# epam/Zstandard

Hardware: NVIDIA B200
Metric: decompress_GBps_uncompressed (higher is better)
Workload: dtype u8

## Files before the change

### zstandard_b200/csrc/decode_kernels.cu

```cuda
#include "zb_decode.cuh"
#include "decode_kernels.cuh"
#include "xxh_device.cuh"
#ifdef ZB_EXEC_DEBUG
#include <stdio.h>
#endif

namespace zb {

__device__ __forceinline__ u64 frame_dst_off(const DecodeArgs& a, u32 f, const FrameInfo& fi) { return a.dst_off[f] + fi.out_base; }
__device__ __forceinline__ u32 frame_cap(const DecodeArgs& a, u32 f, const FrameInfo& fi) { return a.dst_cap[f] - fi.out_base; }
__device__ __forceinline__ u8* lit_region(const DecodeArgs& a, u32 f, const FrameInfo& fi) { return a.lit_arena + (frame_dst_off(a, f, fi) & ~15ull) + 64ull * (a.item_base + f); }
__device__ __forceinline__ u64 lit_capacity(u32 cap) { return (u64)cap + 40; }
__device__ __forceinline__ SeqRec* seq_region(const DecodeArgs& a, u32 f, const FrameInfo& fi) { return a.seq_arena + 2 * (frame_dst_off(a, f, fi) / 3) + 32ull * (a.item_base + f); }

__device__ __forceinline__ u64 unit_slice_base(const DecodeArgs& a) { return a.dst_off[0] / PAR_UNIT_BYTES + (u64)PAR_UNIT_SLACK * a.item_base; }

__device__ __forceinline__ int parse_one(const DecodeArgs& a, u32 i) {
  FrameInfo fi; u32 r = 0; u32 start = 0, outBase = 0;
  if (a.pass) {
    const FrameInfo prev = a.info[i];
    if ((prev.flags & FI_DONE) || prev.next_off == 0 || is_err(a.result[i])) { a.info[i].flags = FI_DONE; return -1; }
    start = prev.next_off; outBase = prev.out_base + prev.decoded;
  }
  const u8* src = a.src_base + a.src_off[i];
// ... 120 lines not shown
          if (ok) ok = huf_build_tables(sm, slot, sub, gmask, body, bodySize, fullMem, T, &hdr);
          if (ok) { body += hdr; bodySize -= hdr; haveTable = true; }
        }
        if (ok) {
          bool good = true;
          if (lh.single) {
            if (sub == 0) good = dry ? huf_check_stream(body, bodySize, lh.litSize, T)
                                     : huf_decode_stream(body, bodySize, lit + litRun, lh.litSize, T, &sm.ring[lane][0]);
          } else {
            HufStream st;
            good = huf_split4(body, bodySize, lh.litSize, sub, st);
            if (good) good = dry ? huf_check_stream(st.src, st.len, st.count, T)
                                 : huf_decode_stream(st.src, st.len, lit + litRun + st.outOfs, st.count, T, &sm.ring[lane][0]);
          }
          unsigned okmask = __ballot_sync(gmask, good);
          if ((okmask & gmask) != gmask) ok = false;
          __syncwarp(gmask);
        }
        if (!ok || dry) { errBlock = blk; errCode = ok ? HUF_DRY : ZE_corruption_detected; break; }
        litRun += lh.litSize;
      }
    }
    pos += bh.csize; blk++;
    if (bh.last) break;
  }
  if (sub == 0 && errBlock != 0xFFFFFFFFu) { a.info[f].huf_err_block = errBlock; a.info[f].huf_err_code = errCode; }
}

template <int R>
__global__ void __launch_bounds__(32) k_huf(DecodeArgs a) {
  extern __shared__ __align__(16) unsigned char smem_raw[];
  HufSmem<R>& sm = *reinterpret_cast<HufSmem<R>*>(smem_raw);
  const u32 lane = threadIdx.x, slot = lane >> 2;
  const u32 nSmall = a.cnt[2];
  if (R == (int)HUF_ROOT_SMALL ? nSmall == 0 : nSmall == a.n) return;
  u16* const fullMem = a.huf_full + (size_t)(blockIdx.x * 8 + slot) * HUF_FULL_STRIDE;
  for (u32 g = blockIdx.x; g * 8 < a.n; g += gridDim.x) {
    const u32 f = g * 8 + slot;
    if (f < a.n) huf_frame(a, sm, f, lane, fullMem);
  }
}

template <int CL, int CO, int CM> struct SeqSmemT {
  u16 ll[1 << CL][32];
  u16 ml[1 << CM][32];
  u16 of[1 << CO][32];
  u16 defLL[64], defOF[32], defML[64];
  u32 llInfo[36], mlInfo[53];
  s16 norm[53][32];
  u16 next[53][32];
  __align__(16) u32 ring[32][ZB_RING_WORDS + 4];
};
typedef SeqSmemT<9, 8, 9> SeqSmem;

template <class SM>
__device__ __forceinline__ void seq_smem_init(SM& sm, u32 lane) {
  if (lane < 3) {
    s16* norm = &sm.norm[0][lane]; u16* next = &sm.next[0][lane];
    Strided<s16> nv{norm, 32}; Strided<u16> sn{next, 32};
    if (lane == 0) { for (int i = 0; i < 36; i++) nv[i] = kLLnorm[i]; build_seq_table(sm.defLL, 1, nv, 35, 6, sn); }
    if (lane == 1) { for (int i = 0; i < 29; i++) nv[i] = kOFnorm[i]; build_seq_table(sm.defOF, 1, nv, 28, 5, sn); }
    if (lane == 2) { for (int i = 0; i < 53; i++) nv[i] = kMLnorm[i]; build_seq_table(sm.defML, 1, nv, 52, 6, sn); }
  }
  for (u32 i = lane; i < 36; i += 32) sm.llInfo[i] = ll_info(i);
  for (u32 i = lane; i < 53; i += 32) sm.mlInfo[i] = ml_info(i);
  __syncwarp();
}

template <int CLS, int CL, int CO, int CM>
__global__ void __launch_bounds__(32) k_seq_t(DecodeArgs a) {
  extern __shared__ __align__(16) unsigned char smem_raw[];
  typedef SeqSmemT<CL, CO, CM> SM;
  SM& sm = *reinterpret_cast<SM*>(smem_raw);
  const u32 lane = threadIdx.x;
  const u32 k = CLS == 0 ? 2 : CLS - 1;
  const u32 count = a.cnt[3 + k];
  if (blockIdx.x * 32 >= count) return;
  seq_smem_init(sm, lane);
  const u32 e = blockIdx.x * 32 + lane;
  if (e >= count) return;
  const u32 f = a.par_list[(size_t)(1 + k) * a.list_stride + a.item_base + e];
  const FrameInfo fi = a.info[f];
  SeqTableSet T;
  T.cap[KIND_LL] = CL; T.cap[KIND_OF] = CO; T.cap[KIND_ML] = CM;
  T.space[KIND_LL] = &sm.ll[0][lane]; T.space[KIND_ML] = &sm.ml[0][lane]; T.space[KIND_OF] = &sm.of[0][lane]; T.stride = 32;
  T.defs[KIND_LL] = sm.defLL; T.defs[KIND_OF] = sm.defOF; T.defs[KIND_ML] = sm.defML;
  SeqEmitter em;
  em.init(seq_region(a, f, fi), seq_capacity(frame_cap(a, f, fi)), sm.llInfo, sm.mlInfo);
  if (a.dict) em.set_reps(a.dict->rep);
  seq_decode_frame(a.src_base + a.src_off[f], a.src_size[f], fi.body_off, fi.window, T, em, sm.llInfo, sm.mlInfo,
                   Strided<s16>{&sm.norm[0][lane], 32}, Strided<u16>{&sm.next[0][lane], 32}, &sm.ring[lane][0], a.dict);
  if (CLS != 0 && em.deferred) {
    a.info[f].flags = fi.flags & ~(u32)(FI_SEQ_A | FI_SEQ_B);
    a.par_list[(size_t)3 * a.list_stride + a.item_base + atomicAdd(a.cnt + 5, 1u)] = f;
    return;
  }
  if (em.res.err_block != 0xFFFFFFFFu) {
    a.info[f].seq_err_block = em.res.err_block; a.info[f].seq_err_code = em.res.err_code; a.info[f].seq_err_index = em.res.err_index;
  }
}

__device__ __forceinline__ void warp_copy(u8* dst, const u8* src, u32 n, u32 lane) {
  if (n < 128) { for (u32 i = lane; i < n; i += 32) dst[i] = src[i]; return; }
  u32 head = (u32)(-(intptr_t)dst) & 15;
  if (lane < head) dst[lane] = src[lane];
  dst += head; src += head; n -= head;
  u32 body = n & ~15u;
  if ((((uintptr_t)src) & 15) == 0) {
    const uint4* s = (const uint4*)src; uint4* d = (uint4*)dst;
    for (u32 i = lane; i < body / 16; i += 32) d[i] = s[i];
  } else {
    const u32 sh = ((u32)(uintptr_t)src & 3) * 8;
    const u32* s = (const u32*)((uintptr_t)src & ~(uintptr_t)3); uint4* d = (uint4*)dst;
    for (u32 i = lane; i < body / 16; i += 32) {
      const u32* p = s + 4 * i;
      u32 w0 = p[0], w1 = p[1], w2 = p[2], w3 = p[3], w4 = sh ? p[4] : 0;
      d[i] = make_uint4(__funnelshift_r(w0, w1, sh), __funnelshift_r(w1, w2, sh), __funnelshift_r(w2, w3, sh), __funnelshift_r(w3, w4, sh));
    }
  }
  for (u32 i = body + lane; i < n; i += 32) dst[i] = src[i];
}
__device__ __forceinline__ void warp_fill(u8* dst, u8 v, u32 n, u32 lane) {
  if (n < 128) { for (u32 i = lane; i < n; i += 32) dst[i] = v; return; }
  u32 head = (u32)(-(intptr_t)dst) & 15;
  if (lane < head) dst[lane] = v;
  dst += head; n -= head;
  u32 body = n & ~15u, w = v * 0x01010101u;
  uint4* d = (uint4*)dst; uint4 vv = make_uint4(w, w, w, w);
  for (u32 i = lane; i < body / 16; i += 32) d[i] = vv;
  for (u32 i = body + lane; i < n; i += 32) dst[i] = v;
}

// ... 309 lines not shown
__global__ void __launch_bounds__(32) k_huf_blk(DecodeArgs a) {
  extern __shared__ __align__(16) unsigned char smem_raw[];
  HufSmem<HUF_TABLE_LOG>& sm = *reinterpret_cast<HufSmem<HUF_TABLE_LOG>*>(smem_raw);
  const u32 lane = threadIdx.x, sub = lane & 3, slot = lane >> 2;
  const unsigned gmask = 0xFu << (slot * 4);
  const u32 nunits = a.cnt[0];
  BlockUnit* const sliceUnits = a.units + unit_slice_base(a);
  u16* const fullMem = a.huf_full + (size_t)(blockIdx.x * 8 + slot) * HUF_FULL_STRIDE;
  for (u32 w0 = blockIdx.x * 8; w0 < nunits; w0 += gridDim.x * 8) {
    const u32 w = w0 + slot;
    if (w >= nunits) continue;
    const BlockUnit u = sliceUnits[w];
    const u32 f = u.frame;
    const FrameInfo fi = a.info[f];
    const u8* src = a.src_base + a.src_off[f];
    const u8* bp = src + u.body;
    LitHdr lh; bool needs;
    read_lit_hdr(bp, u.csize, lh, &needs);
    if (lh.type < 2) continue;
    u8* lit = lit_region(a, f, fi) + u.lit_off;
    bool ok = true;
    HufTabs T{sm.root[slot], HUF_TABLE_LOG, nullptr, nullptr, 0};
    const u8* body = bp + lh.lhSize; u32 bodySize = lh.litCSize;
    __syncwarp(gmask);
    if (lh.type == 3 && u.huf_def == DEF_DICT) huf_dict_tables(sm, slot, sub, gmask, a.dict, T);
    else {
      const u8* tb = body; u32 tbSize = bodySize;
      if (lh.type == 3) {
        const BlockUnit d = sliceUnits[fi.unit_base + u.huf_def];
        LitHdr lhD; bool n2;
        read_lit_hdr(src + d.body, d.csize, lhD, &n2);
        tb = src + d.body + lhD.lhSize; tbSize = lhD.litCSize;
      } else if (!lh.single && (lh.litSize == 0 || bodySize == 0)) ok = false;
      u32 hdr = 0;
      if (ok) ok = huf_build_tables(sm, slot, sub, gmask, tb, tbSize, fullMem, T, &hdr);
      if (ok && lh.type == 2) { body += hdr; bodySize -= hdr; }
    }
    if (ok) {
      bool good = true;
      if (lh.single) {
        if (sub == 0) good = huf_decode_stream(body, bodySize, lit, lh.litSize, T, &sm.ring[lane][0]);
      } else {
        HufStream st;
        good = huf_split4(body, bodySize, lh.litSize, sub, st);
        if (good) good = huf_decode_stream(st.src, st.len, lit + st.outOfs, st.count, T, &sm.ring[lane][0]);
      }
      const unsigned okmask = __ballot_sync(gmask, good);
      if ((okmask & gmask) != gmask) ok = false;
    }
    if (sub == 0 && !ok) sliceUnits[w].huf_err = ZE_corruption_detected;
  }
}

__global__ void __launch_bounds__(32) k_seq_blk(DecodeArgs a) {
  extern __shared__ __align__(16) unsigned char smem_raw[];
  SeqSmem& sm = *reinterpret_cast<SeqSmem*>(smem_raw);
  const u32 lane = threadIdx.x;
  const u32 nunits = a.cnt[0];
  if (blockIdx.x * 32 >= nunits) return;
  if (lane < 3) {
    s16* norm = &sm.norm[0][lane]; u16* next = &sm.next[0][lane];
    Strided<s16> nv{norm, 32}; Strided<u16> sn{next, 32};
    if (lane == 0) { for (int i = 0; i < 36; i++) nv[i] = kLLnorm[i]; build_seq_table(sm.defLL, 1, nv, 35, 6, sn); }
    if (lane == 1) { for (int i = 0; i < 29; i++) nv[i] = kOFnorm[i]; build_seq_table(sm.defOF, 1, nv, 28, 5, sn); }
    if (lane == 2) { for (int i = 0; i < 53; i++) nv[i] = kMLnorm[i]; build_seq_table(sm.defML, 1, nv, 52, 6, sn); }
  }
  for (u32 i = lane; i < 36; i += 32) sm.llInfo[i] = ll_info(i);
  for (u32 i = lane; i < 53; i += 32) sm.mlInfo[i] = ml_info(i);
  __syncwarp();
  BlockUnit* const sliceUnits = a.units + unit_slice_base(a);
  for (u32 w = blockIdx.x * 32 + lane; w < nunits; w += gridDim.x * 32) {
    const BlockUnit u = sliceUnits[w];
    const u32 f = u.frame;
    const FrameInfo fi = a.info[f];
    SeqTableSet T;
    T.space[KIND_LL] = &sm.ll[0][lane]; T.space[KIND_ML] = &sm.ml[0][lane]; T.space[KIND_OF] = &sm.of[0][lane]; T.stride = 32;
    T.defs[KIND_LL] = sm.defLL; T.defs[KIND_OF] = sm.defOF; T.defs[KIND_ML] = sm.defML;
    UnitEmitter em;
    em.init(seq_region(a, f, fi) + u.rec_off, sm.llInfo, sm.mlInfo);
    seq_decode_unit(a.src_base + a.src_off[f], u, sliceUnits + fi.unit_base, fi.window, T, em, sm.llInfo, sm.mlInfo,
                    Strided<s16>{&sm.norm[0][lane], 32}, Strided<u16>{&sm.next[0][lane], 32}, &sm.ring[lane][0], a.dict);
    if (em.dead) { sliceUnits[w].seq_err_code = em.err_code; sliceUnits[w].seq_err_index = em.err_index; }
    else if (em.n) {
      sliceUnits[w].rep[0] = em.h.v0; sliceUnits[w].rep[1] = em.h.v1; sliceUnits[w].rep[2] = em.h.v2;
      sliceUnits[w].rep_sym = em.h.t0 | (em.h.t1 << 3) | (em.h.t2 << 6);
    }
  }
}

#ifndef EXECB_SLEEP
#define EXECB_SLEEP 100
#endif
__host__ __device__ inline u32 execb_warps(u32 npar) { return npar <= 148 * 7 ? 4 : (npar <= 148 * 16 ? 2 : 1); }
template <int W> struct ExecBigShared {
  volatile u32 wm;
  volatile u32 done;
  volatile u32 errG;
  volatile u32 flag[4 * W];
  volatile u32 endPos[4 * W];
  u32 errAt[W], errCode[W];
  volatile u32 left;
  u32 hashed; u64 hv[4];
};
template <int W>
__device__ __forceinline__ void chain_publish(ExecBigShared<W>& sh, u32 G, u32 endPos, u32 lane) {
  __threadfence_block();
  __syncwarp();
  if (lane == 0) {
    if (W == 1) { sh.wm = endPos; sh.done = G + 1; }
    else {
      sh.endPos[G % (4 * W)] = endPos;
      __threadfence_block();
      sh.flag[G % (4 * W)] = G + 1;
      __threadfence_block();
      u32 d = sh.done;
      while (sh.flag[d % (4 * W)] == d + 1) {
        const u32 e = sh.endPos[d % (4 * W)];
        if (atomicCAS((u32*)&sh.done, d, d + 1) == d) atomicMax((u32*)&sh.wm, e);
        __threadfence_block();
        d = sh.done;
      }
    }
  }
  __syncwarp();
// ... 271 lines not shown
      }
      a.result[f] = res;
      a.info[f].trailer_off = trailer; a.info[f].decoded = (u32)op; a.info[f].next_off = nextOff;
      a.info[f].flags = fi.flags | (needXxh ? FI_NEED_XXH : 0);
      if (nextOff && a.more) atomicAdd(a.more, 1u);
    }
  }
}

__global__ void __launch_bounds__(128) k_xxh(DecodeArgs a) {
  const u32 t = blockIdx.x * blockDim.x + threadIdx.x;
  const u32 f = t >> 2, sub = t & 3, lane = threadIdx.x & 31;
  const unsigned gmask = 0xFu << (lane & ~3u);
  if (f >= a.n) return;
  FrameInfo fi = a.info[f];
  if (!(fi.flags & FI_NEED_XXH) || (fi.flags & FI_PAR)) return;
  const u8* dst = a.dst_base + frame_dst_off(a, f, fi);
  u64 h = xxh64_group<false>(dst, fi.decoded, sub, gmask, lane & ~3u);
  if (sub == 0) {
    const u8* src = a.src_base + a.src_off[f];
    if ((u32)h != ld32(src + fi.trailer_off)) a.result[f] = zerr(ZE_checksum_wrong);
  }
}
__global__ void __launch_bounds__(32) k_xxh_big(DecodeArgs a) {
  const u32 lane = threadIdx.x, sub = lane & 3, slot = lane >> 2;
  const unsigned gmask = 0xFu << (lane & ~3u);
  const u32 npar = a.cnt[1];
  for (u32 p = blockIdx.x * 8 + slot; p < npar; p += gridDim.x * 8) {
    const u32 f = a.par_list[a.item_base + p];
    const FrameInfo fi = a.info[f];
    if (!(fi.flags & FI_NEED_XXH)) continue;
    const u8* dst = a.dst_base + frame_dst_off(a, f, fi);
    const u64 h = xxh64_group<true>(dst, fi.decoded, sub, gmask, lane & ~3u);
    if (sub == 0) {
      const u8* src = a.src_base + a.src_off[f];
      if ((u32)h != ld32(src + fi.trailer_off)) a.result[f] = zerr(ZE_checksum_wrong);
    }
  }
}


size_t decode_lit_arena_bytes(u64 max_dst_bytes, u64 max_items) { return (size_t)(max_dst_bytes + 64 * (max_items + 2) + 256); }
size_t decode_seq_arena_bytes(u64 max_dst_bytes, u64 max_items) { return (size_t)((2 * (max_dst_bytes / 3) + 32 * (max_items + 2) + 64) * sizeof(SeqRec)); }

__global__ void __launch_bounds__(32) k_dict(const u8* dict, u32 size, DictState* ds) {
  __shared__ HufBuildWk wk; __shared__ HufFseScratch fs; __shared__ u8 slot[260]; __shared__ s16 norm[64]; __shared__ u16 next[64];
  if (threadIdx.x == 0) dict_load(dict, size, *ds, wk, fs, slot, norm, next);
}
cudaError_t decode_load_dictionary(const u8* d_dict_bytes, u32 size, DictState* d_state, cudaStream_t st) {
  k_dict<<<1, 32, 0, st>>>(d_dict_bytes, size, d_state);
  return cudaGetLastError();
}

static int g_par_grid_huf = 148 * 5, g_grid_huf_small = 148 * 11, g_par_grid_seq = 148 * 2, g_par_grid_exec = 148 * 32;
int decode_huf_ctas() { return g_grid_huf_small > g_par_grid_huf ? g_grid_huf_small : g_par_grid_huf; }
size_t decode_unit_arena_count(u64 max_dst_bytes, u64 max_items) { return (size_t)(max_dst_bytes / PAR_UNIT_BYTES + PAR_UNIT_SLACK * (max_items + 2) + 64); }

cudaError_t decode_configure() {
  cudaError_t e = cudaFuncSetAttribute(k_huf<HUF_TABLE_LOG>, cudaFuncAttributeMaxDynamicSharedMemorySize, (int)sizeof(HufSmem<HUF_TABLE_LOG>));
  if (e != cudaSuccess) return e;
  e = cudaFuncSetAttribute(k_huf<HUF_ROOT_SMALL>, cudaFuncAttributeMaxDynamicSharedMemorySize, (int)sizeof(HufSmem<HUF_ROOT_SMALL>));
  if (e != cudaSuccess) return e;
  e = cudaFuncSetAttribute(k_huf_blk, cudaFuncAttributeMaxDynamicSharedMemorySize, (int)sizeof(HufSmem<HUF_TABLE_LOG>));
  if (e != cudaSuccess) return e;
  e = cudaFuncSetAttribute(k_seq_blk, cudaFuncAttributeMaxDynamicSharedMemorySize, (int)sizeof(SeqSmem));
  if (e != cudaSuccess) return e;
  int dev = 0, sms = 0;
  if (cudaGetDevice(&dev) == cudaSuccess && cudaDeviceGetAttribute(&sms, cudaDevAttrMultiProcessorCount, dev) == cudaSuccess && sms > 0) {
    int per = 0;
    if (cudaOccupancyMaxActiveBlocksPerMultiprocessor(&per, k_huf_blk, 32, sizeof(HufSmem<HUF_TABLE_LOG>)) == cudaSuccess && per > 0) g_par_grid_huf = sms * per;
    if (cudaOccupancyMaxActiveBlocksPerMultiprocessor(&per, k_huf<HUF_ROOT_SMALL>, 32, sizeof(HufSmem<HUF_ROOT_SMALL>)) == cudaSuccess && per > 0) g_grid_huf_small = sms * per;
    if (cudaOccupancyMaxActiveBlocksPerMultiprocessor(&per, k_seq_blk, 32, sizeof(SeqSmem)) == cudaSuccess && per > 0) g_par_grid_seq = sms * per;
    g_par_grid_exec = sms * 32;
  }
  e = cudaFuncSetAttribute(k_seq_t<2, 8, 8, 8>, cudaFuncAttributeMaxDynamicSharedMemorySize, (int)sizeof(SeqSmemT<8, 8, 8>));
  if (e != cudaSuccess) return e;
  return cudaFuncSetAttribute(k_seq_t<0, 9, 8, 9>, cudaFuncAttributeMaxDynamicSharedMemorySize, (int)sizeof(SeqSmem));
}

const char* const kDecodeKernelNames[DECODE_KERNELS] = {"k_parse", "k_huf", "k_seq", "k_exec", "k_xxh"};

cudaError_t decode_launch_entropy(const DecodeArgs& a, cudaStream_t st, int* launches, cudaEvent_t* marks) {
  if (a.n == 0) return cudaSuccess;
  { cudaError_t e = cudaMemsetAsync(a.cnt, 0, 32, st); if (e != cudaSuccess) return e; }
  if (marks) cudaEventRecord(marks[0], st);
  k_parse<<<(a.n + 127) / 128, 128, 0, st>>>(a);
  if (marks) cudaEventRecord(marks[1], st);
  { const u32 need = (a.n + 7) / 8;
    k_huf<HUF_ROOT_SMALL><<<need < (u32)g_grid_huf_small ? need : (u32)g_grid_huf_small, 32, sizeof(HufSmem<HUF_ROOT_SMALL>), st>>>(a);
    k_huf<HUF_TABLE_LOG><<<need < (u32)g_par_grid_huf ? need : (u32)g_par_grid_huf, 32, sizeof(HufSmem<HUF_TABLE_LOG>), st>>>(a); }
  if (a.units) k_huf_blk<<<g_par_grid_huf, 32, sizeof(HufSmem<HUF_TABLE_LOG>), st>>>(a);
  if (marks) cudaEventRecord(marks[2], st);
  k_seq_t<1, 6, 6, 7><<<(a.n + 31) / 32, 32, sizeof(SeqSmemT<6, 6, 7>), st>>>(a);
  k_seq_t<2, 8, 8, 8><<<(a.n + 31) / 32, 32, sizeof(SeqSmemT<8, 8, 8>), st>>>(a);
  k_seq_t<0, 9, 8, 9><<<(a.n + 31) / 32, 32, sizeof(SeqSmem), st>>>(a);
  if (a.units) k_seq_blk<<<g_par_grid_seq, 32, sizeof(SeqSmem), st>>>(a);
  if (marks) cudaEventRecord(marks[3], st);
  if (launches) *launches += a.units ? 8 : 6;
  return cudaGetLastError();
}
cudaError_t decode_launch_exec(const DecodeArgs& a, cudaStream_t st, int* launches, cudaEvent_t* marks) {
  if (a.n == 0) return cudaSuccess;
  if (a.dict) k_exec<true><<<(a.n + (EXEC_THREADS / 32) - 1) / (EXEC_THREADS / 32), EXEC_THREADS, 0, st>>>(a);
  else k_exec<false><<<(a.n + (EXEC_THREADS / 32) - 1) / (EXEC_THREADS / 32), EXEC_THREADS, 0, st>>>(a);
  if (a.units) {
    if (a.dict) {
      k_exec_big<true, 4><<<g_par_grid_exec / 32 * 7, 160, 0, st>>>(a); k_exec_big<true, 2><<<g_par_grid_exec / 2, 64, 0, st>>>(a); k_exec_big<true, 1><<<g_par_grid_exec, 32, 0, st>>>(a);
    } else {
      k_exec_big<false, 4><<<g_par_grid_exec / 32 * 7, 160, 0, st>>>(a); k_exec_big<false, 2><<<g_par_grid_exec / 2, 64, 0, st>>>(a); k_exec_big<false, 1><<<g_par_grid_exec, 32, 0, st>>>(a);
    }
  }
  if (marks) cudaEventRecord(marks[4], st);
  k_xxh<<<(a.n * 4 + 127) / 128, 128, 0, st>>>(a);
  if (a.units) k_xxh_big<<<148 * 8, 32, 0, st>>>(a);
  if (marks) cudaEventRecord(marks[5], st);
  if (launches) *launches += a.units ? 6 : 2;
  return cudaGetLastError();
}
cudaError_t decode_launch(const DecodeArgs& a, cudaStream_t st, int* launches, cudaEvent_t* marks) {
  cudaError_t e = decode_launch_entropy(a, st, launches, marks);
  if (e != cudaSuccess) return e;
  return decode_launch_exec(a, st, launches, marks);
}

}
```

### zstandard_b200/csrc/zb_blocks.cuh

```cuda
#pragma once
#include "zb_decode.cuh"

namespace zb {

enum : u32 { DEF_SELF = 0xFFFFFFFEu, DEF_DICT = 0xFFFFFFFDu, DEF_NONE = 0xFFFFFFFFu };

#define PAR_UNIT_BYTES 16384u
#define PAR_UNIT_SLACK 2u

struct BlockUnit {
  u32 frame;
  u32 body;
  u32 csize;
  u32 lit_off;
  u32 rec_off;
  u32 huf_def;
  u32 tab_def[3];
  u32 huf_err;
  u32 seq_err_code, seq_err_index;
  u32 rep[3];
  u32 rep_sym;
};
static_assert(sizeof(BlockUnit) == 64, "BlockUnit layout");

// ... 89 lines not shown
        if (lh.type == 3) u.huf_def = lastHuf; else lastHuf = n;
        litRun += lh.litSize;
      }
      if (nbSeq) {
        const int kinds[3] = {KIND_LL, KIND_OF, KIND_ML};
        const u32 modeOf[3] = {(modes >> 4) & 3, (modes >> 2) & 3, modes & 3};
        for (int k = 0; k < 3; k++) {
          if (modeOf[k] == 3) { if (lastTab[kinds[k]] == DEF_NONE) return 0; u.tab_def[kinds[k]] = lastTab[kinds[k]]; }
          else lastTab[kinds[k]] = n;
        }
        recRun += 1 + (u64)nbSeq;
        if (recRun > recCap) return 0;
      }
      if (units) units[n] = u;
      n++;
    }
    pos += bh.csize;
    if (bh.last) break;
  }
  return n >= 2 ? n : 0;
}

template <class NormT>
ZB_HD bool unit_locate_table(const u8* bp, u32 bsz, int kind, NormT norm, const u8** desc, u32* descSize, u32* mode) {
  LitHdr lh; bool needs;
  if (read_lit_hdr(bp, bsz, lh, &needs)) return false;
  const u8* sp = bp + lh.consumed; const u32 ssz = bsz - lh.consumed;
  u32 nbSeq, modes, hdr;
  if (read_seq_count(sp, ssz, &nbSeq, &modes, &hdr) || !nbSeq) return false;
  const int kinds[3] = {KIND_LL, KIND_OF, KIND_ML};
  const u32 modeOf[3] = {(modes >> 4) & 3, (modes >> 2) & 3, modes & 3};
  for (int k = 0; k < 3; k++) {
    if (kinds[k] == kind) { *desc = sp + hdr; *descSize = ssz - hdr; *mode = modeOf[k]; return true; }
    if (modeOf[k] == 1) { if (ssz - hdr == 0) return false; hdr += 1; }
    else if (modeOf[k] == 2) {
      u32 max = kinds[k] == KIND_LL ? MaxLL : (kinds[k] == KIND_ML ? MaxML : MaxOff), tl, h;
      if (read_ncount(norm, &max, &tl, sp + hdr, ssz - hdr, &h)) return false;
      hdr += h;
    }
  }
  return false;
}

template <class NormT, class NextT>
ZB_HD void seq_decode_unit(const u8* src, const BlockUnit& u, const BlockUnit* frameUnits, u64 window, SeqTableSet& T, UnitEmitter& em,
                           const u32* llInfo, const u32* mlInfo, NormT norm, NextT symbolNext, u32* ringMem, const DictState* dict) {
  const u8* bp = src + u.body; const u32 bsz = u.csize;
  LitHdr lh; bool needs;
  read_lit_hdr(bp, bsz, lh, &needs);
  const u8* sp = bp + lh.consumed; const u32 ssz = bsz - lh.consumed;
  u32 nbSeq, modes, hdr;
  read_seq_count(sp, ssz, &nbSeq, &modes, &hdr);
  if (!nbSeq) return;
  for (int k = 0; k < 3; k++) { T.cur[k] = T.space[k]; T.curStride[k] = T.stride; T.log[k] = 0; }
  const int kinds[3] = {KIND_LL, KIND_OF, KIND_ML};
  const u32 modeOf[3] = {(modes >> 4) & 3, (modes >> 2) & 3, modes & 3};
  u32 e = 0;
  for (int k = 0; k < 3 && !e; k++) {
    const int kind = kinds[k]; u32 used = 0, lg = 0; bool isDef = false;
    if (modeOf[k] == 3) continue;
    e = read_seq_table(modeOf[k], kind, sp + hdr, ssz - hdr, T.space[kind], T.stride, &lg, &isDef, true, &used, norm, symbolNext);
    if (!e) { hdr += used; T.log[kind] = lg; if (isDef) { T.cur[kind] = T.defs[kind]; T.curStride[kind] = 1; } }
  }
  for (int k = 0; k < 3 && !e; k++) {
    const int kind = kinds[k];
    if (modeOf[k] != 3) continue;
    const u32 def = u.tab_def[kind];
    if (def == DEF_DICT) {
      const u32 cells = 1u << dict->log[kind];
      for (u32 c = 0; c < cells; c++) T.space[kind][c * T.stride] = dict->cells[kind][c];
      T.log[kind] = dict->log[kind];
    } else {
      const BlockUnit& d = frameUnits[def];
      const u8* desc; u32 descSize, mode, used = 0, lg = 0; bool isDef = false;
      if (!unit_locate_table(src + d.body, d.csize, kind, norm, &desc, &descSize, &mode)) { e = ZE_corruption_detected; break; }
      e = read_seq_table(mode, kind, desc, descSize, T.space[kind], T.stride, &lg, &isDef, true, &used, norm, symbolNext);
      if (!e) { T.log[kind] = lg; if (isDef) { T.cur[kind] = T.defs[kind]; T.curStride[kind] = 1; } }
    }
  }
  if (e) { em.fail(0, ZE_corruption_detected); return; }
  seq_decode_bitstream(sp + hdr, ssz - hdr, nbSeq, window, T, em, llInfo, mlInfo, ringMem, 0);
}

}
```

### zstandard_b200/csrc/zb_decode.cuh

```cuda
#pragma once
#include "zb_format.cuh"

namespace zb {

struct alignas(16) SeqRec { u32 x, y, z, w; };
ZB_HD void rec_store(SeqRec* p, u32 x, u32 y, u32 z, u32 w) {
#if defined(__CUDA_ARCH__)
  *reinterpret_cast<uint4*>(p) = make_uint4(x, y, z, w);
#else
  p->x = x; p->y = y; p->z = z; p->w = w;
#endif
}
ZB_HD u32 rec_ll(const SeqRec& r) { return r.w & 0x1FFFF; }
ZB_HD u32 rec_ml(const SeqRec& r) { return (r.w >> 17) | (((r.y >> 18) & 7) << 15); }
ZB_HD u32 rec_lpos(const SeqRec& r) { return r.y & 0x3FFFF; }
ZB_HD u32 sat_add32(u32 a, u32 b) { const u32 s = a + b; return s < a ? 0xFFFFFFFFu : s; }
ZB_HD u32 sat_lpos(u32 lpos, u32 ll) { const u32 s = lpos + ll; return s > 0x3FFFFu ? 0x3FFFFu : s; }

ZB_HD u64 seq_capacity(u64 cap) { return 2 * (cap / 3) + 24; }

struct SeqTableSet {
  u32 cap[3] = {9, 9, 9};
  u16* space[3];
  u32 stride;
  const u16* defs[3];
  const u16* cur[3]; u32 curStride[3]; u32 log[3];
};

struct SeqFrameOut {
  u32 err_block, err_code, err_index;
};

ZB_HD u32 top_bits(u64 w, u32 n) { return (u32)((w >> 1) >> (63 - n)); }

ZB_HD u32 rep_resolve(u32& rep0, u32& rep1, u32& rep2, u32 ofBits, u32 ofv, u32 llSym) {
  const bool isRep = ofBits <= 1;
  const u32 raw = (1u << (ofBits & 31)) - 3 + ofv;
  const u32 idx = ofBits + ofv + (llSym == 0);
  u32 pick = rep0;
  pick = idx == 1 ? rep1 : pick;
  pick = idx == 2 ? rep2 : pick;
  pick = idx == 3 ? rep0 - 1 : pick;
  pick = pick == 0 ? 1 : pick;
  const u32 offset = isRep ? pick : raw;
  const bool keep1 = isRep && idx == 0;
  const bool keep2 = isRep && idx <= 1;
  const u32 n2 = keep2 ? rep2 : rep1, n1 = keep1 ? rep1 : rep0;
  rep2 = n2; rep1 = n1; rep0 = offset;
  return offset;
}

struct RefBits {
  const u8* s; u32 n;
  i32 k;
  u32 bc, C;
};
ZB_HD void refbits_load(RefBits& b) {
  if (b.n >= 4) { b.C = ld32(b.s + b.k); return; }
  b.C = b.s[0]; if (b.n >= 2) b.C |= (u32)b.s[1] << 8; if (b.n >= 3) b.C |= (u32)b.s[2] << 16;
}
ZB_HD void refbits_at(RefBits& b, const u8* s, u32 n, i32 P) {
  b.s = s; b.n = n;
  const i32 bcn = (8 - (P & 7)) & 7, above = P - 32 + bcn;
  if (n >= 4 && above >= 0) { b.k = above >> 3; b.bc = (u32)bcn; } else { b.k = 0; b.bc = (u32)(32 - P); }
  refbits_load(b);
}
ZB_HD u32 refbits_read_fast(RefBits& b, u32 nb) { u32 v = (b.C << (b.bc & 31)) >> ((32 - nb) & 31); b.bc += nb; return v; }
ZB_HD void refbits_reload(RefBits& b) {
  if (b.bc > 32 || b.k == 0) return;
  u32 nb = b.bc >> 3;
  if (b.k >= 4 || (i32)nb <= b.k) { b.k -= (i32)nb; b.bc -= nb * 8; } else { b.bc -= (u32)b.k * 8; b.k = 0; }
  refbits_load(b);
}
ZB_HD void seq_values_ref32(const u8* s, u32 n, i32 P, bool longOffsets, bool longVariant, u32 ofBits, u32 mlBits, u32 llBits, u32& ofv, u32& mlv, u32& llv) {
  RefBits b; refbits_at(b, s, n, P);
  ofv = 0;
  if (ofBits) {
    if (longOffsets && (longVariant || ofBits >= 25)) {
      const u32 room = longVariant ? 24 : 32 - b.bc, extra = ofBits - (ofBits < room ? ofBits : room);
      ofv = refbits_read_fast(b, ofBits - extra) << (extra & 31);
// ... 6 lines not shown
  llv = llBits ? refbits_read_fast(b, llBits) : 0;
}

struct SeqEmitter {
  SeqRec* out; u32 cap; const u32* llInfo; const u32* mlInfo;
  u32 n;
  u32 hdrSlot, dpos, lpos;
  u32 rep0, rep1, rep2;
  bool dead;
  bool deferred;
  SeqFrameOut res;
  ZB_HD void init(SeqRec* o, u64 cap64, const u32* lli, const u32* mli) {
    out = o; cap = (u32)cap64; llInfo = lli; mlInfo = mli;
    n = 0; hdrSlot = 0; dpos = 0; lpos = 0; rep0 = 1; rep1 = 4; rep2 = 8; dead = false; deferred = false;
    res.err_block = 0xFFFFFFFFu; res.err_code = 0; res.err_index = 0;
  }
  ZB_HD void set_reps(const u32* r) { rep0 = r[0]; rep1 = r[1]; rep2 = r[2]; }
  ZB_HD void block_begin() { if (dead) return; hdrSlot = n++; dpos = 0; lpos = 0; }
  ZB_HD void emit(u32 ofBits, u32 ofv, u32 llSym, u32 ll, u32 ml) {
    const u32 offset = rep_resolve(rep0, rep1, rep2, ofBits, ofv, llSym);
    if (n < cap) rec_store(out + n, dpos, lpos | ((ml >> 15) << 18), offset, ll | (ml << 17));
    n++; dpos = sat_add32(dpos, ll + ml); lpos = sat_lpos(lpos, ll);
  }
  ZB_HD void fast(u32 hi, u32 llSym, u32 ofBits, u32 iLL, u32 iML) {
    const u32 llBits = iLL >> 24, mlBits = iML >> 24;
    const u32 ofv = shr_c(hi, 32 - ofBits);
    const u32 mlv = shr_c(hi << ofBits, 32 - mlBits);
    const u32 llv = shr_c(hi << (ofBits + mlBits), 32 - llBits);
    emit(ofBits, ofv, llSym, (iLL & 0xFFFFFF) + llv, (iML & 0xFFFFFF) + mlv);
  }
  ZB_HD void values(u32 ofv, u32 mlv, u32 llv, u32 llSym, u32 mlSym, u32 ofBits) {
    emit(ofBits, ofv, llSym, (llInfo[llSym] & 0xFFFFFF) + llv, (mlInfo[mlSym] & 0xFFFFFF) + mlv);
  }
  ZB_HD bool stopped() const { return dead; }
  ZB_HD void defer() { deferred = true; }
  ZB_HD void block_end(u32 blk, u32 runnable, bool bad) {
    if (dead) return;
    const bool overflow = n > cap;
    u32 count = (overflow ? cap : n) - hdrSlot - 1;
    if (bad && runnable < count) count = runnable;
    if (hdrSlot < cap) rec_store(out + hdrSlot, count, dpos, lpos, 0);
    if (overflow) { res.err_block = blk; res.err_code = ZE_dstSize_tooSmall; res.err_index = 0; dead = true; }
    else if (bad) { res.err_block = blk; res.err_code = ZE_corruption_detected; res.err_index = runnable; dead = true; }
  }
  ZB_HD void fail(u32 blk, u32 code) { if (dead) return; res.err_block = blk; res.err_code = code; res.err_index = 0xFFFFFFFFu; dead = true; }
};

template <class Sink>
ZB_HD bool seq_decode_bitstream(const u8* bits, u32 nbytes, u32 nbSeq, u64 window, const SeqTableSet& T, Sink& sink,
                                const u32* llInfo, const u32* mlInfo, u32* ringMem, u32 blk) {
  bool longVariant = false;
  if (window > (1u << 24)) {
    const u32 lg = T.log[KIND_OF]; u32 total = 0;
    for (u32 u = 0; u < (1u << lg); u++) total += (T.cur[KIND_OF][u * T.curStride[KIND_OF]] >> 10) > 22;
    longVariant = (total << (8 - lg)) >= 20;
  }
  BitCursor c;
  sink.block_begin();
  u32 decoded = 0; bool bad = false;
  if (!bc_init(c, bits, nbytes)) bad = true;
  if (!bad) {
    i32 P = c.P;
    const u16 *tLL = T.cur[KIND_LL], *tOF = T.cur[KIND_OF], *tML = T.cur[KIND_ML];
    const u32 sLLs = T.curStride[KIND_LL], sOFs = T.curStride[KIND_OF], sMLs = T.curStride[KIND_ML];
    u32 stLL, stOF, stML;
    { u64 w = bc_window64(c, P); u32 lg = T.log[KIND_LL]; stLL = top_bits(w, lg); w <<= lg; P -= (i32)lg;
      lg = T.log[KIND_OF]; stOF = top_bits(w, lg); w <<= lg; P -= (i32)lg;
      lg = T.log[KIND_ML]; stML = top_bits(w, lg); P -= (i32)lg; }
    u32 i = 0;
    BitRing ring;
    if (nbSeq && P >= 128) ring_init(ring, ringMem, bits, nbytes);
    while (i < nbSeq && P >= 128) {
      u32 lo, hi;
      ring_window(ring, P, lo, hi);
      const u32 yLL = tLL[stLL * sLLs], yOF = tOF[stOF * sOFs], yML = tML[stML * sMLs];
      const u32 llSym = yLL >> 10, mlSym = yML >> 10, ofBits = yOF >> 10;
      const u32 iLL = llInfo[llSym], iML = mlInfo[mlSym];
      const u32 valBits = ofBits + (iML >> 24) + (iLL >> 24);
      const u32 lLL = yLL & 0x3FF, lOF = yOF & 0x3FF, lML = yML & 0x3FF;
      const u32 nLL = cell_nb(lLL), nML = cell_nb(lML), nOF = cell_nb(lOF);
      if (valBits >= 32) break;
      sink.fast(hi, llSym, ofBits, iLL, iML);
      const u32 h2 = fshl(lo, hi, valBits);
      stLL = cell_base(lLL) + shr_c(h2, 32 - nLL);
      stML = cell_base(lML) + shr_c(h2 << nLL, 32 - nML);
      stOF = cell_base(lOF) + shr_c(h2 << (nLL + nML), 32 - nOF);
      const i32 Pn = P - (i32)(valBits + nLL + nML + nOF);
      ring_advance(ring, Pn);
      P = Pn; i++;
    }
    decoded = i;
    for (; i < nbSeq; i++) {
      if (P < 0) { bad = true; break; }
      const u64 w0 = bc_window64(c, P);
      const u32 yLL = tLL[stLL * sLLs], yOF = tOF[stOF * sOFs], yML = tML[stML * sMLs];
      const u32 llSym = yLL >> 10, mlSym = yML >> 10, ofBits = yOF >> 10;
      const u32 llBits = llInfo[llSym] >> 24, mlBits = mlInfo[mlSym] >> 24;
      const u32 lLL = yLL & 0x3FF, lOF = yOF & 0x3FF, lML = yML & 0x3FF;
      const u32 nLL = cell_nb(lLL), nML = cell_nb(lML), nOF = cell_nb(lOF);
      const u32 valBits = ofBits + mlBits + llBits, stBits = nLL + nML + nOF;
      u64 w = w0;
      u32 ofv = top_bits(w, ofBits); w <<= ofBits;
      u32 mlv = top_bits(w, mlBits); w <<= mlBits;
      u32 llv = top_bits(w, llBits); w <<= llBits;
      const i32 Pv = P - (i32)valBits;
      if (Pv < 0) seq_values_ref32(bits, nbytes, P, window > (1ull << 25), longVariant, ofBits, mlBits, llBits, ofv, mlv, llv);
      else if (valBits + stBits > 64) w = bc_window64(c, Pv);
      sink.values(ofv, mlv, llv, llSym, mlSym, ofBits);
      decoded++;
      stLL = cell_base(lLL) + top_bits(w, nLL); w <<= nLL;
      stML = cell_base(lML) + top_bits(w, nML); w <<= nML;
      stOF = cell_base(lOF) + top_bits(w, nOF);
      P = Pv - (i32)stBits;
    }
  }
  if (bad && longVariant) decoded = decoded > 4 ? decoded - 4 : 0;
  sink.block_end(blk, decoded, bad);
  return bad || sink.stopped();
}

template <class Sink, class NormT, class NextT>
ZB_HD void seq_decode_frame(const u8* src, u32 size, u32 body_off, u64 window, SeqTableSet& T, Sink& sink,
                            const u32* llInfo, const u32* mlInfo, NormT norm, NextT symbolNext, u32* ringMem, const DictState* dict = nullptr) {
  u32 pos = body_off, blk = 0;
  bool haveRepeat = false;
  for (int k = 0; k < 3; k++) { T.cur[k] = T.space[k]; T.curStride[k] = T.stride; T.log[k] = 0; }
  if (dict && dict->hasEntropy) {
    for (int k = 0; k < 3; k++) {
      const u32 n = 1u << dict->log[k];
      for (u32 u = 0; u < n; u++) T.space[k][u * T.stride] = dict->cells[k][u];
      T.log[k] = dict->log[k];
    }
    haveRepeat = true;
  }
  while (true) {
    BlockHdr bh;
    if (read_block_hdr(src + pos, size - pos, bh)) return;
    pos += 3;
    if (bh.type == 2) {
      const u8* bp = src + pos; u32 bsz = bh.csize;
      if (bsz >= BLOCKSIZE_MAX) return;
      LitHdr lh; bool needs;
      if (read_lit_hdr(bp, bsz, lh, &needs)) return;
      const u8* sp = bp + lh.consumed; u32 ssz = bsz - lh.consumed;
      u32 nbSeq, modes, hdr;
      u32 e = read_seq_count(sp, ssz, &nbSeq, &modes, &hdr);
      if (e) { sink.fail(blk, e); return; }
      if (nbSeq) {
        const int kinds[3] = {KIND_LL, KIND_OF, KIND_ML};
        const u32 modeOf[3] = {(modes >> 4) & 3, (modes >> 2) & 3, modes & 3};
        for (int k = 0; k < 3 && !e; k++) {
          int kind = kinds[k]; u32 used, lg = T.log[kind]; bool isDef = false;
          u32 m = modeOf[k];
          e = read_seq_table(m, kind, sp + hdr, ssz - hdr, T.space[kind], T.stride, &lg, &isDef, haveRepeat, &used, norm, symbolNext, T.cap[kind]);
          if (e == ZB_TABLE_TOO_LARGE) { sink.defer(); return; }
          if (!e) {
            hdr += used;
            if (m != 3) {
              T.log[kind] = lg;
              if (isDef) { T.cur[kind] = T.defs[kind]; T.curStride[kind] = 1; }
              else { T.cur[kind] = T.space[kind]; T.curStride[kind] = T.stride; }
            }
          }
        }
        if (e) { sink.fail(blk, ZE_corruption_detected); return; }
        haveRepeat = true;
        if (seq_decode_bitstream(sp + hdr, ssz - hdr, nbSeq, window, T, sink, llInfo, mlInfo, ringMem, blk)) return;
      }
    }
    pos += bh.csize; blk++;
    if (bh.last) return;
  }
}

struct HufStream { const u8* src; u32 len; u32 outOfs; u32 count; };

ZB_HD bool huf_split4(const u8* body, u32 bodySize, u32 n, u32 lane, HufStream& s) {
  if (bodySize < 10) return false;
  u32 l1 = ld16(body), l2 = ld16(body + 2), l3 = ld16(body + 4);
  u32 l4 = bodySize - (l1 + l2 + l3 + 6);
  if (l4 > bodySize) return false;
  u32 seg = (n + 3) / 4;
  u32 start = 6, len = l1;
  if (lane == 1) { start = 6 + l1; len = l2; } else if (lane == 2) { start = 6 + l1 + l2; len = l3; } else if (lane == 3) { start = 6 + l1 + l2 + l3; len = l4; }
  s.src = body + start; s.len = len; s.outOfs = lane * seg;
  s.count = lane < 3 ? seg : (n > 3 * seg ? n - 3 * seg : 0);
  return true;
}

struct HufTabs { const u16* root; u32 rootLog; const u16* full; const u8* side; u32 log; };
template <bool LONGS>
ZB_HD u32 huf_cell(const HufTabs& T, u64 w) {
  u32 c = T.root[(u32)(w >> (64 - T.rootLog))];
  if (LONGS && c >= HUF_LONG) {
    if (T.log > HUF_TABLE_LOG) { const u32 i12 = (u32)(w >> 52), cell = T.full[i12 >> 1]; c = (cell >> 8) == 12 ? (12u << 8) | T.side[i12] : cell; }
    else c = T.full[(u32)(w >> (64 - T.log))];
  }
  return c;
}
template <bool LONGS>
ZB_HD u32 huf_cell32(const HufTabs& T, u32 w32) {
  u32 c = T.root[w32 >> (32 - T.rootLog)];
  if (LONGS && c >= HUF_LONG) c = huf_cell<true>(T, (u64)w32 << 32);
  return c;
}

template <bool LONGS>
ZB_HD bool huf_decode_stream_t(const u8* src, u32 len, u8* out, u32 count, const HufTabs& T, u32* ringMem) {
  BitCursor c;
  if (!bc_init(c, src, len)) return false;
  i32 P = c.P;
  u32 left = count;
  while (left && ((uintptr_t)out & 3)) {
    const u32 cell = huf_cell<LONGS>(T, bc_window64(c, P));
    *out++ = (u8)cell; P -= (i32)(cell >> 8); left--;
// ... 50 lines not shown
```

Before: 207.2.

## Pack many seq-decode warps per CTA, copy predefined tables, pipeline FSE loop

The sequence-decode kernels now launch CTAs holding as many warps as fit in 227KB of shared memory, each warp using its own slice, instead of one 32-thread CTA per warp. Predefined FSE tables are copied into the per-lane strided table space, which drops the per-kind cur pointer and stride indirection. The fast sequence loop is software-pipelined: the next state's table loads and the ring window refill are issued before the sink emits the current sequence. Together these aim to cut launch and CTA-scheduling overhead and shorten the serial dependency chain, at the cost of extra copies when predefined tables are used and a fixed per-SM residency.

```diff
diff --git a/zstandard_b200/csrc/decode_kernels.cu b/zstandard_b200/csrc/decode_kernels.cu
--- a/zstandard_b200/csrc/decode_kernels.cu
+++ b/zstandard_b200/csrc/decode_kernels.cu
@@ -196,6 +196,9 @@
   __align__(16) u32 ring[32][ZB_RING_WORDS + 4];
 };
 typedef SeqSmemT<9, 8, 9> SeqSmem;
+template <class SM> __host__ __device__ constexpr int seq_cta_warps() { return (int)((227u << 10) / sizeof(SM)); }
+template <class SM> constexpr size_t seq_cta_smem() { return seq_cta_warps<SM>() * sizeof(SM); }
+template <class SM> constexpr u32 seq_grid(u32 n) { return (n + 32 * seq_cta_warps<SM>() - 1) / (32 * seq_cta_warps<SM>()); }
 
 template <class SM>
 __device__ __forceinline__ void seq_smem_init(SM& sm, u32 lane) {
@@ -212,16 +215,16 @@
 }
 
 template <int CLS, int CL, int CO, int CM>
-__global__ void __launch_bounds__(32) k_seq_t(DecodeArgs a) {
+__global__ void __launch_bounds__(32 * seq_cta_warps<SeqSmemT<CL, CO, CM>>(), 1) k_seq_t(DecodeArgs a) {
   extern __shared__ __align__(16) unsigned char smem_raw[];
   typedef SeqSmemT<CL, CO, CM> SM;
-  SM& sm = *reinterpret_cast<SM*>(smem_raw);
-  const u32 lane = threadIdx.x;
+  const u32 lane = threadIdx.x & 31, warp = blockIdx.x * seq_cta_warps<SM>() + (threadIdx.x >> 5);
+  SM& sm = reinterpret_cast<SM*>(smem_raw)[threadIdx.x >> 5];
   const u32 k = CLS == 0 ? 2 : CLS - 1;
   const u32 count = a.cnt[3 + k];
-  if (blockIdx.x * 32 >= count) return;
+  if (warp * 32 >= count) return;
   seq_smem_init(sm, lane);
-  const u32 e = blockIdx.x * 32 + lane;
+  const u32 e = warp * 32 + lane;
   if (e >= count) return;
   const u32 f = a.par_list[(size_t)(1 + k) * a.list_stride + a.item_base + e];
   const FrameInfo fi = a.info[f];
@@ -637,12 +640,12 @@
   }
 }
 
-__global__ void __launch_bounds__(32) k_seq_blk(DecodeArgs a) {
+__global__ void __launch_bounds__(32 * seq_cta_warps<SeqSmem>(), 1) k_seq_blk(DecodeArgs a) {
   extern __shared__ __align__(16) unsigned char smem_raw[];
-  SeqSmem& sm = *reinterpret_cast<SeqSmem*>(smem_raw);
-  const u32 lane = threadIdx.x;
+  SeqSmem& sm = reinterpret_cast<SeqSmem*>(smem_raw)[threadIdx.x >> 5];
+  const u32 lane = threadIdx.x & 31, warp = blockIdx.x * seq_cta_warps<SeqSmem>() + (threadIdx.x >> 5);
   const u32 nunits = a.cnt[0];
-  if (blockIdx.x * 32 >= nunits) return;
+  if (warp * 32 >= nunits) return;
   if (lane < 3) {
     s16* norm = &sm.norm[0][lane]; u16* next = &sm.next[0][lane];
     Strided<s16> nv{norm, 32}; Strided<u16> sn{next, 32};
@@ -654,7 +657,7 @@
   for (u32 i = lane; i < 53; i += 32) sm.mlInfo[i] = ml_info(i);
   __syncwarp();
   BlockUnit* const sliceUnits = a.units + unit_slice_base(a);
-  for (u32 w = blockIdx.x * 32 + lane; w < nunits; w += gridDim.x * 32) {
+  for (u32 w = warp * 32 + lane; w < nunits; w += gridDim.x * blockDim.x) {
     const BlockUnit u = sliceUnits[w];
     const u32 f = u.frame;
     const FrameInfo fi = a.info[f];
@@ -1032,7 +1035,7 @@
   return cudaGetLastError();
 }
 
-static int g_par_grid_huf = 148 * 5, g_grid_huf_small = 148 * 11, g_par_grid_seq = 148 * 2, g_par_grid_exec = 148 * 32;
+static int g_par_grid_huf = 148 * 5, g_grid_huf_small = 148 * 11, g_par_grid_seq = 148, g_par_grid_exec = 148 * 32;
 int decode_huf_ctas() { return g_grid_huf_small > g_par_grid_huf ? g_grid_huf_small : g_par_grid_huf; }
 size_t decode_unit_arena_count(u64 max_dst_bytes, u64 max_items) { return (size_t)(max_dst_bytes / PAR_UNIT_BYTES + PAR_UNIT_SLACK * (max_items + 2) + 64); }
 
@@ -1043,19 +1046,22 @@
   if (e != cudaSuccess) return e;
   e = cudaFuncSetAttribute(k_huf_blk, cudaFuncAttributeMaxDynamicSharedMemorySize, (int)sizeof(HufSmem<HUF_TABLE_LOG>));
   if (e != cudaSuccess) return e;
-  e = cudaFuncSetAttribute(k_seq_blk, cudaFuncAttributeMaxDynamicSharedMemorySize, (int)sizeof(SeqSmem));
+  e = cudaFuncSetAttribute(k_seq_blk, cudaFuncAttributeMaxDynamicSharedMemorySize, (int)seq_cta_smem<SeqSmem>());
   if (e != cudaSuccess) return e;
   int dev = 0, sms = 0;
   if (cudaGetDevice(&dev) == cudaSuccess && cudaDeviceGetAttribute(&sms, cudaDevAttrMultiProcessorCount, dev) == cudaSuccess && sms > 0) {
     int per = 0;
     if (cudaOccupancyMaxActiveBlocksPerMultiprocessor(&per, k_huf_blk, 32, sizeof(HufSmem<HUF_TABLE_LOG>)) == cudaSuccess && per > 0) g_par_grid_huf = sms * per;
     if (cudaOccupancyMaxActiveBlocksPerMultiprocessor(&per, k_huf<HUF_ROOT_SMALL>, 32, sizeof(HufSmem<HUF_ROOT_SMALL>)) == cudaSuccess && per > 0) g_grid_huf_small = sms * per;
-    if (cudaOccupancyMaxActiveBlocksPerMultiprocessor(&per, k_seq_blk, 32, sizeof(SeqSmem)) == cudaSuccess && per > 0) g_par_grid_seq = sms * per;
+    if (cudaOccupancyMaxActiveBlocksPerMultiprocessor(&per, k_seq_blk, 32 * seq_cta_warps<SeqSmem>(), seq_cta_smem<SeqSmem>()) == cudaSuccess && per > 0)
+      g_par_grid_seq = sms * per;
     g_par_grid_exec = sms * 32;
   }
-  e = cudaFuncSetAttribute(k_seq_t<2, 8, 8, 8>, cudaFuncAttributeMaxDynamicSharedMemorySize, (int)sizeof(SeqSmemT<8, 8, 8>));
+  e = cudaFuncSetAttribute(k_seq_t<1, 6, 6, 7>, cudaFuncAttributeMaxDynamicSharedMemorySize, (int)seq_cta_smem<SeqSmemT<6, 6, 7>>());
   if (e != cudaSuccess) return e;
-  return cudaFuncSetAttribute(k_seq_t<0, 9, 8, 9>, cudaFuncAttributeMaxDynamicSharedMemorySize, (int)sizeof(SeqSmem));
+  e = cudaFuncSetAttribute(k_seq_t<2, 8, 8, 8>, cudaFuncAttributeMaxDynamicSharedMemorySize, (int)seq_cta_smem<SeqSmemT<8, 8, 8>>());
+  if (e != cudaSuccess) return e;
+  return cudaFuncSetAttribute(k_seq_t<0, 9, 8, 9>, cudaFuncAttributeMaxDynamicSharedMemorySize, (int)seq_cta_smem<SeqSmem>());
 }
 
 const char* const kDecodeKernelNames[DECODE_KERNELS] = {"k_parse", "k_huf", "k_seq", "k_exec", "k_xxh"};
@@ -1071,10 +1077,10 @@
     k_huf<HUF_TABLE_LOG><<<need < (u32)g_par_grid_huf ? need : (u32)g_par_grid_huf, 32, sizeof(HufSmem<HUF_TABLE_LOG>), st>>>(a); }
   if (a.units) k_huf_blk<<<g_par_grid_huf, 32, sizeof(HufSmem<HUF_TABLE_LOG>), st>>>(a);
   if (marks) cudaEventRecord(marks[2], st);
-  k_seq_t<1, 6, 6, 7><<<(a.n + 31) / 32, 32, sizeof(SeqSmemT<6, 6, 7>), st>>>(a);
-  k_seq_t<2, 8, 8, 8><<<(a.n + 31) / 32, 32, sizeof(SeqSmemT<8, 8, 8>), st>>>(a);
-  k_seq_t<0, 9, 8, 9><<<(a.n + 31) / 32, 32, sizeof(SeqSmem), st>>>(a);
-  if (a.units) k_seq_blk<<<g_par_grid_seq, 32, sizeof(SeqSmem), st>>>(a);
+  k_seq_t<1, 6, 6, 7><<<seq_grid<SeqSmemT<6, 6, 7>>(a.n), 32 * seq_cta_warps<SeqSmemT<6, 6, 7>>(), seq_cta_smem<SeqSmemT<6, 6, 7>>(), st>>>(a);
+  k_seq_t<2, 8, 8, 8><<<seq_grid<SeqSmemT<8, 8, 8>>(a.n), 32 * seq_cta_warps<SeqSmemT<8, 8, 8>>(), seq_cta_smem<SeqSmemT<8, 8, 8>>(), st>>>(a);
+  k_seq_t<0, 9, 8, 9><<<seq_grid<SeqSmem>(a.n), 32 * seq_cta_warps<SeqSmem>(), seq_cta_smem<SeqSmem>(), st>>>(a);
+  if (a.units) k_seq_blk<<<g_par_grid_seq, 32 * seq_cta_warps<SeqSmem>(), seq_cta_smem<SeqSmem>(), st>>>(a);
   if (marks) cudaEventRecord(marks[3], st);
   if (launches) *launches += a.units ? 8 : 6;
   return cudaGetLastError();
diff --git a/zstandard_b200/csrc/zb_blocks.cuh b/zstandard_b200/csrc/zb_blocks.cuh
--- a/zstandard_b200/csrc/zb_blocks.cuh
+++ b/zstandard_b200/csrc/zb_blocks.cuh
@@ -165,7 +165,7 @@
   u32 nbSeq, modes, hdr;
   read_seq_count(sp, ssz, &nbSeq, &modes, &hdr);
   if (!nbSeq) return;
-  for (int k = 0; k < 3; k++) { T.cur[k] = T.space[k]; T.curStride[k] = T.stride; T.log[k] = 0; }
+  for (int k = 0; k < 3; k++) T.log[k] = 0;
   const int kinds[3] = {KIND_LL, KIND_OF, KIND_ML};
   const u32 modeOf[3] = {(modes >> 4) & 3, (modes >> 2) & 3, modes & 3};
   u32 e = 0;
@@ -173,7 +173,7 @@
     const int kind = kinds[k]; u32 used = 0, lg = 0; bool isDef = false;
     if (modeOf[k] == 3) continue;
     e = read_seq_table(modeOf[k], kind, sp + hdr, ssz - hdr, T.space[kind], T.stride, &lg, &isDef, true, &used, norm, symbolNext);
-    if (!e) { hdr += used; T.log[kind] = lg; if (isDef) { T.cur[kind] = T.defs[kind]; T.curStride[kind] = 1; } }
+    if (!e) { hdr += used; if (isDef) seq_use_predefined(T, kind, lg); else T.log[kind] = lg; }
   }
   for (int k = 0; k < 3 && !e; k++) {
     const int kind = kinds[k];
@@ -188,7 +188,7 @@
       const u8* desc; u32 descSize, mode, used = 0, lg = 0; bool isDef = false;
       if (!unit_locate_table(src + d.body, d.csize, kind, norm, &desc, &descSize, &mode)) { e = ZE_corruption_detected; break; }
       e = read_seq_table(mode, kind, desc, descSize, T.space[kind], T.stride, &lg, &isDef, true, &used, norm, symbolNext);
-      if (!e) { T.log[kind] = lg; if (isDef) { T.cur[kind] = T.defs[kind]; T.curStride[kind] = 1; } }
+      if (!e) { if (isDef) seq_use_predefined(T, kind, lg); else T.log[kind] = lg; }
     }
   }
   if (e) { em.fail(0, ZE_corruption_detected); return; }
diff --git a/zstandard_b200/csrc/zb_decode.cuh b/zstandard_b200/csrc/zb_decode.cuh
--- a/zstandard_b200/csrc/zb_decode.cuh
+++ b/zstandard_b200/csrc/zb_decode.cuh
@@ -24,8 +24,12 @@
   u16* space[3];
   u32 stride;
   const u16* defs[3];
-  const u16* cur[3]; u32 curStride[3]; u32 log[3];
+  u32 log[3];
 };
+ZB_HD void seq_use_predefined(SeqTableSet& T, int kind, u32 lg) {
+  for (u32 u = 0; u < (1u << lg); u++) T.space[kind][u * T.stride] = T.defs[kind][u];
+  T.log[kind] = lg;
+}
 
 struct SeqFrameOut {
   u32 err_block, err_code, err_index;
@@ -138,7 +142,7 @@
   bool longVariant = false;
   if (window > (1u << 24)) {
     const u32 lg = T.log[KIND_OF]; u32 total = 0;
-    for (u32 u = 0; u < (1u << lg); u++) total += (T.cur[KIND_OF][u * T.curStride[KIND_OF]] >> 10) > 22;
+    for (u32 u = 0; u < (1u << lg); u++) total += (T.space[KIND_OF][u * T.stride] >> 10) > 22;
     longVariant = (total << (8 - lg)) >= 20;
   }
   BitCursor c;
@@ -147,39 +151,48 @@
   if (!bc_init(c, bits, nbytes)) bad = true;
   if (!bad) {
     i32 P = c.P;
-    const u16 *tLL = T.cur[KIND_LL], *tOF = T.cur[KIND_OF], *tML = T.cur[KIND_ML];
-    const u32 sLLs = T.curStride[KIND_LL], sOFs = T.curStride[KIND_OF], sMLs = T.curStride[KIND_ML];
+    const u16 *tLL = T.space[KIND_LL], *tOF = T.space[KIND_OF], *tML = T.space[KIND_ML];
+    const u32 ts = T.stride;
     u32 stLL, stOF, stML;
     { u64 w = bc_window64(c, P); u32 lg = T.log[KIND_LL]; stLL = top_bits(w, lg); w <<= lg; P -= (i32)lg;
       lg = T.log[KIND_OF]; stOF = top_bits(w, lg); w <<= lg; P -= (i32)lg;
       lg = T.log[KIND_ML]; stML = top_bits(w, lg); P -= (i32)lg; }
     u32 i = 0;
-    BitRing ring;
-    if (nbSeq && P >= 128) ring_init(ring, ringMem, bits, nbytes);
-    while (i < nbSeq && P >= 128) {
+    if (nbSeq && P >= 128) {
+      BitRing ring;
+      ring_init(ring, ringMem, bits, nbytes);
       u32 lo, hi;
       ring_window(ring, P, lo, hi);
-      const u32 yLL = tLL[stLL * sLLs], yOF = tOF[stOF * sOFs], yML = tML[stML * sMLs];
-      const u32 llSym = yLL >> 10, mlSym = yML >> 10, ofBits = yOF >> 10;
-      const u32 iLL = llInfo[llSym], iML = mlInfo[mlSym];
-      const u32 valBits = ofBits + (iML >> 24) + (iLL >> 24);
-      const u32 lLL = yLL & 0x3FF, lOF = yOF & 0x3FF, lML = yML & 0x3FF;
-      const u32 nLL = cell_nb(lLL), nML = cell_nb(lML), nOF = cell_nb(lOF);
-      if (valBits >= 32) break;
-      sink.fast(hi, llSym, ofBits, iLL, iML);
-      const u32 h2 = fshl(lo, hi, valBits);
-      stLL = cell_base(lLL) + shr_c(h2, 32 - nLL);
-      stML = cell_base(lML) + shr_c(h2 << nLL, 32 - nML);
-      stOF = cell_base(lOF) + shr_c(h2 << (nLL + nML), 32 - nOF);
-      const i32 Pn = P - (i32)(valBits + nLL + nML + nOF);
-      ring_advance(ring, Pn);
-      P = Pn; i++;
+      u32 yLL = tLL[stLL * ts], yOF = tOF[stOF * ts], yML = tML[stML * ts];
+      u32 iLL = llInfo[yLL >> 10], iML = mlInfo[yML >> 10];
+      u32 valBits, h2, nLL, nML, nOF;
+      auto chain_in = [&]() {
+        valBits = (yOF >> 10) + (iML >> 24) + (iLL >> 24);
+        h2 = fshl(lo, hi, valBits);
+        nLL = cell_nb(yLL & 0x3FF); nML = cell_nb(yML & 0x3FF); nOF = cell_nb(yOF & 0x3FF);
+      };
+      chain_in();
+      if (valBits < 32) while (true) {
+        const u32 sLL = cell_base(yLL & 0x3FF) + shr_c(h2, 32 - nLL);
+        const u32 sML = cell_base(yML & 0x3FF) + shr_c(h2 << nLL, 32 - nML);
+        const u32 sOF = cell_base(yOF & 0x3FF) + shr_c(h2 << (nLL + nML), 32 - nOF);
+        const i32 Pn = P - (i32)(valBits + nLL + nML + nOF);
+        const u32 llSym = yLL >> 10, ofBits = yOF >> 10, v = hi, jLL = iLL, jML = iML;
+        yLL = tLL[sLL * ts]; yOF = tOF[sOF * ts]; yML = tML[sML * ts];
+        ring_advance(ring, Pn);
+        ring_window(ring, Pn, lo, hi);
+        iLL = llInfo[yLL >> 10]; iML = mlInfo[yML >> 10];
+        sink.fast(v, llSym, ofBits, jLL, jML);
+        stLL = sLL; stML = sML; stOF = sOF; P = Pn; i++;
+        chain_in();
+        if (i >= nbSeq || P < 128 || valBits >= 32) break;
+      }
     }
     decoded = i;
     for (; i < nbSeq; i++) {
       if (P < 0) { bad = true; break; }
       const u64 w0 = bc_window64(c, P);
-      const u32 yLL = tLL[stLL * sLLs], yOF = tOF[stOF * sOFs], yML = tML[stML * sMLs];
+      const u32 yLL = tLL[stLL * ts], yOF = tOF[stOF * ts], yML = tML[stML * ts];
       const u32 llSym = yLL >> 10, mlSym = yML >> 10, ofBits = yOF >> 10;
       const u32 llBits = llInfo[llSym] >> 24, mlBits = mlInfo[mlSym] >> 24;
       const u32 lLL = yLL & 0x3FF, lOF = yOF & 0x3FF, lML = yML & 0x3FF;
@@ -210,7 +223,7 @@
                             const u32* llInfo, const u32* mlInfo, NormT norm, NextT symbolNext, u32* ringMem, const DictState* dict = nullptr) {
   u32 pos = body_off, blk = 0;
   bool haveRepeat = false;
-  for (int k = 0; k < 3; k++) { T.cur[k] = T.space[k]; T.curStride[k] = T.stride; T.log[k] = 0; }
+  for (int k = 0; k < 3; k++) T.log[k] = 0;
   if (dict && dict->hasEntropy) {
     for (int k = 0; k < 3; k++) {
       const u32 n = 1u << dict->log[k];
@@ -242,11 +255,8 @@
           if (e == ZB_TABLE_TOO_LARGE) { sink.defer(); return; }
           if (!e) {
             hdr += used;
-            if (m != 3) {
-              T.log[kind] = lg;
-              if (isDef) { T.cur[kind] = T.defs[kind]; T.curStride[kind] = 1; }
-              else { T.cur[kind] = T.space[kind]; T.curStride[kind] = T.stride; }
-            }
+            if (isDef) seq_use_predefined(T, kind, lg);
+            else if (m != 3) T.log[kind] = lg;
           }
         }
         if (e) { sink.fail(blk, ZE_corruption_detected); return; }
```

Result: faster. 223.0 (median of 6 runs) (+7.6%).
